# taintpro98/rnd-semantic-segmentation

Measured on AMD Instinct MI355X. Metric: train images/sec at 769x769 bf16 (DeepLabV2-ResNet101 + ASPP), higher is better.
Workload: dtype bf16; 1 GPU; train_src.py DeepLabV2-R101 bf16, 769x769 synthetic Cityscapes crops, batch 8 per GPU, 1xMI355X; global_batch=8, parallelism=dp1, weights=formula (synthetic), hip_graph_replay=False

## Files before the change

### rnd_semantic_segmentation_amd/csrc/pack_aspp.hip

```cpp
#include "mi_common.h"

namespace {

__global__ void pack_fwd_kernel(const float* __restrict__ w, __bf16* __restrict__ wp, int O, int I, int T) {
    const long idx = (long)blockIdx.x * blockDim.x + threadIdx.x;
    if (idx >= (long)O * I) return;
    const long plane = (long)O * I;
    for (int t = 0; t < T; ++t) wp[t * plane + idx] = (__bf16)w[idx * T + t];
}

__global__ void pack_dgrad_kernel(const float* __restrict__ w, const float* __restrict__ scale, __bf16* __restrict__ wp, int O, int I, int T) {
    const long idx = (long)blockIdx.x * blockDim.x + threadIdx.x;
    if (idx >= (long)O * I) return;
    const int i = (int)(idx / O), o = (int)(idx - (long)i * O);
    const float s = scale ? scale[o] : 1.f;
    const long plane = (long)O * I;
    const float* src = w + ((long)o * I + i) * T;
    for (int t = 0; t < T; ++t) wp[t * plane + idx] = (__bf16)(src[t] * s);
}

__global__ void aspp_pack_fwd_kernel(const float* __restrict__ w4, __bf16* __restrict__ wall, int C, int K) {
    const long idx = (long)blockIdx.x * blockDim.x + threadIdx.x;
    const long total = 36L * MI_ASPP_ZGW * C;
    if (idx >= total) return;
// ... 9 lines not shown

__global__ void aspp_pack_dgrad_kernel(const float* __restrict__ w4, __bf16* __restrict__ wallT, int C, int K) {
    const long idx = (long)blockIdx.x * blockDim.x + threadIdx.x;
    const long total = (long)C * MI_ASPP_KPAD;
    if (idx >= total) return;
    const int c = (int)(idx / MI_ASPP_KPAD), k = (int)(idx - (long)c * MI_ASPP_KPAD);
    float v = 0.f;
    if (k < 36 * K) {
        const int g = k / K, n = k - g * K;
        const int r = g / 9, tap = g - r * 9;
        v = w4[(((long)r * K + n) * C + c) * 9 + tap];
    }
    wallT[idx] = (__bf16)v;
}

constexpr int PACK_TILES = 4;
__global__ __launch_bounds__(256) void pack_multi_kernel(const float* __restrict__ wflat, const float* __restrict__ sflat, __bf16* __restrict__ wp,
                                                         __bf16* __restrict__ wpt, const long* __restrict__ table, int n_desc) {
    __shared__ float tile[32][32 * 9 + 1];
    int lo = 0, hi = n_desc - 1;
    while (lo < hi) {
        const int mid = (lo + hi + 1) >> 1;
        if (table[mid * 8 + 7] <= (long)blockIdx.x) lo = mid; else hi = mid - 1;
    }
    const long* d = table + lo * 8;
    const int O = (int)d[4], I = (int)d[5], T = (int)d[6];
    const int tiles_i = (I + 31) >> 5, groups_i = (tiles_i + PACK_TILES - 1) / PACK_TILES;
    const int local = (int)((long)blockIdx.x - d[7]);
    const int ot = local / groups_i;
    const int o0 = ot * 32, it0 = (local - ot * groups_i) * PACK_TILES;
    if (o0 >= O) return;
    const int no = min(32, O - o0);
    const int tid = threadIdx.x, lane = tid & 63, wave = tid >> 6;
    const long plane = (long)O * I;
    const int c = tid & 31, r = tid >> 5;
    const float sc = (d[3] >= 0 && d[1] >= 0 && c < no) ? sflat[d[1] + o0 + c] : 1.f;
    for (int it = it0; it < it0 + PACK_TILES && it < tiles_i; ++it) {
        const int i0 = it * 32;
        const int ni = min(32, I - i0);
        const int rowlen = ni * T;
        if (it != it0) __syncthreads();
        for (int o = wave; o < no; o += 4) {
            const float* src = wflat + d[0] + ((long)(o0 + o) * I + i0) * T;
            for (int e = lane; e < rowlen; e += 64) tile[o][e] = src[e];
        }
        __syncthreads();
        if (c < ni) {
            for (int k = 0; k < 4; ++k) {
                const int o = r + 8 * k;
                if (o >= no) break;
                __bf16* f = wp + d[2] + (long)(o0 + o) * I + i0 + c;
                for (int t = 0; t < T; ++t) f[t * plane] = (__bf16)tile[o][c * T + t];
            }
        }
        if (d[3] >= 0 && c < no) {
            for (int k = 0; k < 4; ++k) {
                const int i = r + 8 * k;
                if (i >= ni) break;
                __bf16* b = wpt + d[3] + (long)(i0 + i) * O + o0 + c;
                for (int t = 0; t < T; ++t) b[t * plane] = (__bf16)(tile[c][i * T + t] * sc);
            }
        }
    }
}

struct Rates { int d[4]; };

__global__ void aspp_col2im_kernel(const float* __restrict__ z, const float* __restrict__ bias4, float* __restrict__ low,
                                   int B, int H, int W, int K, Rates rates) {
    const long idx = (long)blockIdx.x * blockDim.x + threadIdx.x;
    const long M = (long)B * H * W;
    if (idx >= M * MI_ASPP_ZGW) return;
    const long m = idx / MI_ASPP_ZGW;
    const int n = (int)(idx - m * MI_ASPP_ZGW);
    if (n >= K) return;
// ... 149 lines not shown
    MI_CHECK_LAUNCH("mi_pack_weight_fwd");
    return MI_OK;
}

extern "C" int mi_pack_weight_dgrad(const float* w, const float* scale_o, void* wp, int O, int I, int ksize, void* stream) {
    MI_REQUIRE(w && wp && O > 0 && I > 0 && ksize > 0, "mi_pack_weight_dgrad: bad argument");
    hipLaunchKernelGGL(pack_dgrad_kernel, dim3(nblk((long)O * I, 256)), dim3(256), 0, (hipStream_t)stream, w, scale_o, (__bf16*)wp, O, I,
                       ksize * ksize);
    MI_CHECK_LAUNCH("mi_pack_weight_dgrad");
    return MI_OK;
}

extern "C" int mi_pack_weights_multi(const float* wflat, const float* sflat, void* wp, void* wpt, const int64_t* table_dev, int n_desc,
                                     int total_blocks, void* stream) {
    MI_REQUIRE(wflat && wp && table_dev && n_desc > 0 && total_blocks > 0, "mi_pack_weights_multi: bad argument");
    hipLaunchKernelGGL(pack_multi_kernel, dim3(total_blocks), dim3(256), 0, (hipStream_t)stream, wflat, sflat, (__bf16*)wp, (__bf16*)wpt,
                       (const long*)table_dev, n_desc);
    MI_CHECK_LAUNCH("mi_pack_weights_multi");
    return MI_OK;
}

extern "C" int mi_aspp_pack_fwd(const float* w4, void* wall, int C, int K, void* stream) {
    MI_REQUIRE(w4 && wall && C > 0 && K > 0 && K < MI_ASPP_ZGW, "mi_aspp_pack_fwd: bad argument (K=%d must be < 20)", K);
    hipLaunchKernelGGL(aspp_pack_fwd_kernel, dim3(nblk(36L * MI_ASPP_ZGW * C, 256)), dim3(256), 0, (hipStream_t)stream, w4, (__bf16*)wall, C, K);
    MI_CHECK_LAUNCH("mi_aspp_pack_fwd");
    return MI_OK;
}

extern "C" int mi_aspp_pack_dgrad(const float* w4, void* wallT, int C, int K, void* stream) {
    MI_REQUIRE(w4 && wallT && C > 0 && K > 0 && 36 * K <= MI_ASPP_KPAD, "mi_aspp_pack_dgrad: bad argument");
    hipLaunchKernelGGL(aspp_pack_dgrad_kernel, dim3(nblk((long)C * MI_ASPP_KPAD, 256)), dim3(256), 0, (hipStream_t)stream, w4, (__bf16*)wallT, C, K);
// ... 38 lines not shown
```

### rnd_semantic_segmentation_amd/csrc/stem.hip

```cpp
#include "mi_common.h"

namespace {

__global__ void stem_pool_fwd_kernel(const bf16x8* __restrict__ y, const float* __restrict__ scale, const float* __restrict__ shift,
                                     bf16x8* __restrict__ pool, uint8_t* __restrict__ idx, int B, int Hc, int Wc, int C8, int Hp, int Wp) {
    const long id = (long)blockIdx.x * blockDim.x + threadIdx.x;
    if (id >= (long)B * Hp * Wp * C8) return;
    const int c8 = (int)(id % C8);
    const int wo = (int)((id / C8) % Wp), ho = (int)((id / ((long)C8 * Wp)) % Hp), b = (int)(id / ((long)C8 * Wp * Hp));
    float sc[8], sh[8], best[8];
    int bi[8];
#pragma unroll
    for (int e = 0; e < 8; ++e) {
        sc[e] = scale[c8 * 8 + e];
        sh[e] = shift[c8 * 8 + e];
        best[e] = -3.0e38f;
        bi[e] = 9;
    }
#pragma unroll
    for (int ky = 0; ky < 3; ++ky) {
        const int h = 2 * ho - 1 + ky;
        if ((unsigned)h >= (unsigned)Hc) continue;
#pragma unroll
        for (int kx = 0; kx < 3; ++kx) {
// ... 38 lines not shown
            const bf16x8 g = dpool[p];
            const uint2 ib = *reinterpret_cast<const uint2*>(idx + p * 8);
#pragma unroll
            for (int e = 0; e < 8; ++e) {
                const unsigned byte = ((e < 4 ? ib.x : ib.y) >> (8 * (e & 3))) & 0xffu;
                if ((int)byte == tap) acc[e] += (float)g[e];
            }
        }
    }
    bf16x8 o;
#pragma unroll
    for (int e = 0; e < 8; ++e) o[e] = (__bf16)(acc[e] * scale[c8 * 8 + e]);
    dy[id] = o;
}

}

extern "C" int mi_stem_pool_fwd(const void* y, const float* scale, const float* shift, void* pool, uint8_t* idx, int B, int Hc, int Wc, int C,
                                int Hp, int Wp, void* stream) {
    MI_REQUIRE(y && scale && shift && pool && idx && B > 0 && Hc > 0 && Wc > 0 && C > 0 && C % 8 == 0, "mi_stem_pool_fwd: bad argument");
    MI_REQUIRE(Hp == (Hc + 2 - 3) / 2 + 1 && Wp == (Wc + 2 - 3) / 2 + 1, "mi_stem_pool_fwd: pooled size must be that of a 3x3/2/1 max-pool");
    MI_REQUIRE(mi_aligned16(y) && mi_aligned16(pool) && ((uintptr_t)idx & 7) == 0, "mi_stem_pool_fwd: alignment");
    const long n = (long)B * Hp * Wp * (C / 8);
    hipLaunchKernelGGL(stem_pool_fwd_kernel, dim3((unsigned)((n + 255) / 256)), dim3(256), 0, (hipStream_t)stream, (const bf16x8*)y, scale, shift,
                       (bf16x8*)pool, idx, B, Hc, Wc, C / 8, Hp, Wp);
    MI_CHECK_LAUNCH("mi_stem_pool_fwd");
    return MI_OK;
}

extern "C" int mi_stem_pool_bwd(const void* dpool, const uint8_t* idx, const float* scale, void* dy, int B, int Hc, int Wc, int C, int Hp, int Wp,
                                void* stream) {
    MI_REQUIRE(dpool && idx && scale && dy && B > 0 && Hc > 0 && Wc > 0 && C > 0 && C % 8 == 0, "mi_stem_pool_bwd: bad argument");
    MI_REQUIRE(Hp == (Hc + 2 - 3) / 2 + 1 && Wp == (Wc + 2 - 3) / 2 + 1, "mi_stem_pool_bwd: pooled size must be that of a 3x3/2/1 max-pool");
    MI_REQUIRE(mi_aligned16(dpool) && mi_aligned16(dy) && ((uintptr_t)idx & 7) == 0, "mi_stem_pool_bwd: alignment");
    const long n = (long)B * Hc * Wc * (C / 8);
    hipLaunchKernelGGL(stem_pool_bwd_kernel, dim3((unsigned)((n + 255) / 256)), dim3(256), 0, (hipStream_t)stream, (const bf16x8*)dpool, idx, scale,
                       (bf16x8*)dy, B, Hc, Wc, C / 8, Hp, Wp);
    MI_CHECK_LAUNCH("mi_stem_pool_bwd");
    return MI_OK;
}

namespace {
__global__ __launch_bounds__(256) void stem_im2col_kernel(const __bf16* __restrict__ x, bf16x8* __restrict__ col, int B, int H, int W, int Ho, int Wo,
                                                          int groups) {
    const int in_row = blockIdx.x * 256 + threadIdx.x;
    if (in_row >= Wo * groups) return;
    const int wo = in_row / groups, kg = in_row - wo * groups;
    const int ho = blockIdx.y % Ho, b = blockIdx.y / Ho;
    int k = kg * 8;
    int c = k / 49, r = k - c * 49, ky = r / 7, kx = r - ky * 7;
    const __bf16* img = x + (long)b * H * W * 3;
    bf16x8 v;
#pragma unroll
    for (int e = 0; e < 8; ++e) {
        __bf16 val = (__bf16)0.f;
        if (k + e < 147) {
            const int h = 2 * ho - 3 + ky, w = 2 * wo - 3 + kx;
            if ((unsigned)h < (unsigned)H && (unsigned)w < (unsigned)W) val = img[((long)h * W + w) * 3 + c];
        }
        v[e] = val;
        if (++kx == 7) {
            kx = 0;
            if (++ky == 7) {
                ky = 0;
                ++c;
            }
        }
    }
    col[((long)blockIdx.y * Wo + wo) * groups + kg] = v;
}
}

extern "C" int mi_stem_im2col(const void* x_bf16_nhwc, void* col_bf16, int B, int H, int W, int Ho, int Wo, int ncols, void* stream) {
    MI_REQUIRE(x_bf16_nhwc && col_bf16 && B > 0 && H > 0 && W > 0, "mi_stem_im2col: bad argument");
    MI_REQUIRE(ncols >= 152 && ncols % 8 == 0 && ncols <= 256, "mi_stem_im2col: ncols=%d (a multiple of 8 in [152, 256])", ncols);
    MI_REQUIRE(Ho == (H + 6 - 7) / 2 + 1 && Wo == (W + 6 - 7) / 2 + 1, "mi_stem_im2col: output size must be that of a 7x7/2/3 conv");
    MI_REQUIRE(mi_aligned16(col_bf16), "mi_stem_im2col: alignment");
    MI_REQUIRE((long)B * Ho < 65536, "mi_stem_im2col: B * Ho = %ld exceeds the grid", (long)B * Ho);
    hipLaunchKernelGGL(stem_im2col_kernel, dim3((unsigned)((Wo * (ncols / 8) + 255) / 256), (unsigned)(B * Ho)), dim3(256), 0, (hipStream_t)stream,
                       (const __bf16*)x_bf16_nhwc, (bf16x8*)col_bf16, B, H, W, Ho, Wo, ncols / 8);
    MI_CHECK_LAUNCH("mi_stem_im2col");
    return MI_OK;
}
```

### rnd_semantic_segmentation_amd/csrc/upsample_ce.hip

```cpp
#include "mi_common.h"

namespace {

constexpr int KMAX = 32;

struct Axis {
    float scale, off;
    int n_in, n_out;
    __device__ __forceinline__ float srcf(int dst) const {
        const float f = scale * ((float)dst + off) - off;
        return f < 0.f ? 0.f : f;
    }
    __device__ __forceinline__ void src(int dst, int& i0, int& i1, float& lam) const {
        const float f = srcf(dst);
        i0 = (int)f;
        if (i0 > n_in - 1) i0 = n_in - 1;
        i1 = (i0 < n_in - 1) ? i0 + 1 : i0;
        lam = f - (float)i0;
    }
    __device__ __forceinline__ int first_with_i0_ge(int c) const {
        if (c <= 0) return 0;
        if (scale <= 0.f) return n_out;
        if (c > n_in - 1) return n_out;
        int d = (int)((float)c / scale) - 2;
// ... 138 lines not shown
    const float* p = logits + b * K * HW + pix;
    float* d = dlogits + b * K * HW + pix;
    if (lab == ignore_index || lab < 0 || lab >= K) {
        for (int k = 0; k < K; ++k) d[k * HW] = 0.f;
        return;
    }
    const float inv = grad_scale / loss_out[1];
    float mx = p[0];
    for (int k = 1; k < K; ++k) mx = fmaxf(mx, p[k * HW]);
    float se = 0.f;
    for (int k = 0; k < K; ++k) se += __expf(p[k * HW] - mx);
    const float rse = 1.f / se;
    for (int k = 0; k < K; ++k) d[k * HW] = (__expf(p[k * HW] - mx) * rse - (k == lab ? 1.f : 0.f)) * inv;
}

constexpr int JT = 32;

template <int KT>
__global__ __launch_bounds__(256) void upce_pass1_kernel(const float* __restrict__ low, const int64_t* __restrict__ labels,
                                                         float* __restrict__ partial, float* __restrict__ tmp, int B, int Krt, Axis ay,
                                                         Axis ax, int ignore_index, int npx_max, unsigned* __restrict__ bad, int jt_cols) {
    const int K = KT > 0 ? KT : Krt;
    constexpr int KR = KT > 0 ? KT : KMAX;
    extern __shared__ __attribute__((aligned(16))) float sh[];
    float* dbuf = sh;
    float* lam = sh + (long)npx_max * K;
    int* x0s = reinterpret_cast<int*>(lam + npx_max);
    float* red = reinterpret_cast<float*>(x0s + npx_max);
    int* pstart = reinterpret_cast<int*>(red + 512);
    float* vrow = red + 512 + JT + 4;
    const int H = ay.n_out, W = ax.n_out, h = ay.n_in, w = ax.n_in;
    const int jt = blockIdx.x, y = blockIdx.y, b = blockIdx.z;
    const int j0 = jt * jt_cols, j1 = min(w, j0 + jt_cols);
    const int xa = ax.first_with_i0_ge(j0 - 1), xb = ax.first_with_i0_ge(j1);
    const int npx = xb - xa;
    int y0, y1;
    float ly;
    ay.src(y, y0, y1, ly);
    const float* row0 = low + ((long)b * h + y0) * w * K;
    const float* row1 = low + ((long)b * h + y1) * w * K;
    const int cbase = max(j0 - 1, 0), ncol = min(j1, w - 1) - cbase + 1;
    if (threadIdx.x < j1 - j0 + 2) pstart[threadIdx.x] = ax.first_with_i0_ge(j0 - 1 + (int)threadIdx.x) - xa;
    for (int e = threadIdx.x; e < ncol * K; e += 256) {
        const long o = (long)cbase * K + e;
        vrow[e] = (1.f - ly) * row0[o] + ly * row1[o];
    }
    __syncthreads();
    float loss = 0.f, cnt = 0.f;
    for (int px = threadIdx.x; px < npx; px += 256) {
        const int x = xa + px;
        int x0, x1;
        float lx;
        ax.src(x, x0, x1, lx);
        lam[px] = lx;
        const long lab = labels[((long)b * H + y) * W + x];
        float* d = dbuf + (long)px * K;
        if (x0 >= j0) count_bad_label(lab, K, ignore_index, bad);
        if (lab == ignore_index || lab < 0 || lab >= K) {
            for (int k = 0; k < K; ++k) d[k] = 0.f;
            continue;
        }
        const float* c0 = vrow + (x0 - cbase) * K;
        const float* c1 = vrow + (x1 - cbase) * K;
        float v[KR];
        float mx = -3.0e38f;
#pragma unroll
        for (int k = 0; k < KR; ++k) {
            if (k < K) {
                v[k] = (1.f - lx) * c0[k] + lx * c1[k];
                mx = fmaxf(mx, v[k]);
// ... 8 lines not shown
                se += v[k];
            }
        }
        const float rse = 1.f / se;
#pragma unroll
        for (int k = 0; k < KR; ++k) {
            if (k < K) d[k] = v[k] * rse - (k == lab ? 1.f : 0.f);
        }
        if (x0 >= j0) {
            loss += __logf(se) - picked;
            cnt += 1.f;
        }
    }
    __syncthreads();
    if (tmp) {
        const int nj = j1 - j0;
        for (int item = threadIdx.x; item < nj * K; item += 256) {
            const int jj = item / K, k = item - jj * K;
            const int j = j0 + jj;
            float s = 0.f;
            const int p0 = max(pstart[jj], 0), p1 = min(max(pstart[jj + 1], 0), npx), p2 = min(pstart[jj + 2], npx);
            for (int px = p0; px < p1; ++px) s += (0.f + lam[px]) * dbuf[(long)px * K + k];
            const bool edge = j == w - 1;
            for (int px = p1; px < p2; ++px) s += ((1.f - lam[px]) + (edge ? lam[px] : 0.f)) * dbuf[(long)px * K + k];
            tmp[(((long)b * H + y) * w + j) * K + k] = s;
        }
    }
    block_sum2(loss, cnt, red);
    if (threadIdx.x == 0) {
        const long pidx = ((long)b * H + y) * gridDim.x + jt;
        partial[2 * pidx] = loss;
        partial[2 * pidx + 1] = cnt;
    }
}

__global__ void upce_pass2_kernel(const float* __restrict__ tmp, const float* __restrict__ loss_out, float* __restrict__ dlow, int B, int K,
                                  Axis ay, int w, float grad_scale) {
    const long idx = (long)blockIdx.x * blockDim.x + threadIdx.x;
    const int H = ay.n_out, h = ay.n_in;
    const long per_row = (long)w * K;
    if (idx >= (long)B * h * per_row) return;
    const long jk = idx % per_row;
    const int i = (int)((idx / per_row) % h), b = (int)(idx / (per_row * h));
// ... 312 lines not shown
}

extern "C" int mi_upsample_ce_ex(const float* low, const int64_t* labels, float* loss_out, float* dlow, int B, int h, int w, int K, int H, int W,
                                 int ignore_index, float grad_scale, int align_corners, void* workspace, size_t workspace_bytes, void* stream) {
    MI_REQUIRE(low && labels && loss_out && workspace, "mi_upsample_ce: null operand");
    MI_REQUIRE(B > 0 && h > 0 && w > 0 && H > 0 && W > 0 && K > 0 && K <= KMAX, "mi_upsample_ce: bad dimension (K <= 32)");
    MI_REQUIRE(H >= h && W >= w, "mi_upsample_ce: only upsampling (H >= h, W >= w) is supported");
    MI_REQUIRE(H <= 65535 && B <= 65535, "mi_upsample_ce: grid dimension overflow");
    if (workspace_bytes < mi_upsample_ce_workspace(B, h, w, K, H, W)) return mi_set_error(MI_ENOMEM, "mi_upsample_ce: workspace too small");
    const Axis ay = make_axis(h, H, align_corners), ax = make_axis(w, W, align_corners);
    const int jt_cols = pick_jt(w, W);
    const int tiles = (w + jt_cols - 1) / jt_cols;
    float* partial = (float*)workspace;
    const size_t poff = (((size_t)B * H * tiles * 2 * sizeof(float)) + 255) & ~(size_t)255;
    float* tmp = dlow ? (float*)((char*)workspace + poff) : nullptr;
    const int npx_max = pass1_npx_max(ax, jt_cols);
    const size_t lds = (size_t)npx_max * K * 4 + (size_t)npx_max * 8 + 512 * 4 + (JT + 4) * 4 + (size_t)(JT + 2) * K * 4;
    MI_REQUIRE(lds <= 160 * 1024, "mi_upsample_ce: upsample factor too large for one LDS tile (%zu B)", lds);
    static std::atomic<uint64_t> lds_set[2];
    mi_allow_dynamic_lds((const void*)upce_pass1_kernel<19>, MI_LDS_MAX, lds_set[0]);
    mi_allow_dynamic_lds((const void*)upce_pass1_kernel<0>, MI_LDS_MAX, lds_set[1]);
    unsigned* bad = reinterpret_cast<unsigned*>(loss_out + 3);
    if (hipMemsetAsync(bad, 0, sizeof(unsigned), (hipStream_t)stream) != hipSuccess) return mi_set_error(MI_EHIP, "mi_upsample_ce: memset");
    if (K == 19)
        hipLaunchKernelGGL(upce_pass1_kernel<19>, dim3(tiles, H, B), dim3(256), lds, (hipStream_t)stream, low, labels, partial, tmp, B, K, ay,
                           ax, ignore_index, npx_max, bad, jt_cols);
    else
        hipLaunchKernelGGL(upce_pass1_kernel<0>, dim3(tiles, H, B), dim3(256), lds, (hipStream_t)stream, low, labels, partial, tmp, B, K, ay,
                           ax, ignore_index, npx_max, bad, jt_cols);
    MI_CHECK_LAUNCH("mi_upsample_ce pass1");
    hipLaunchKernelGGL(ce_finalize_kernel, dim3(1), dim3(256), 0, (hipStream_t)stream, (const float*)partial, B * H * tiles, loss_out);
    MI_CHECK_LAUNCH("mi_upsample_ce finalize");
    if (dlow) {
        hipLaunchKernelGGL(upce_pass2_kernel, dim3(nblk((long)B * h * w * K, 256)), dim3(256), 0, (hipStream_t)stream, (const float*)tmp, loss_out,
                           dlow, B, K, ay, w, grad_scale);
        MI_CHECK_LAUNCH("mi_upsample_ce pass2");
    }
    return MI_OK;
}

extern "C" int mi_upsample_softmax(const float* low, float* probs, uint8_t* pred, int B, int h, int w, int K, int H, int W, void* stream) {
    MI_REQUIRE(low && probs && B > 0 && h > 0 && w > 0 && H > 0 && W > 0 && K > 0 && K <= KMAX, "mi_upsample_softmax: bad argument (K <= 32)");
    hipLaunchKernelGGL(upsample_softmax_kernel, dim3(nblk((long)B * H * W, 256)), dim3(256), 0, (hipStream_t)stream, low, probs, pred, B, K,
                       make_axis(h, H), make_axis(w, W));
// ... 69 lines not shown
```

### rnd_semantic_segmentation_amd/host/engine.py

```python
import contextlib
import os

import torch

from .. import kernels as K
from . import arch


class FlatStore:

    ALIGN = 64

    def __init__(self, named_params, device):
        self.names = [n for n, _ in named_params]
        self.params = [p for _, p in named_params]
        self.offsets = []
        off = 0
        for p in self.params:
            self.offsets.append(off)
            off += -(-p.numel() // self.ALIGN) * self.ALIGN
        self.total = off
        self.data = torch.zeros(off, dtype=torch.float32, device=device)
        self.grad = torch.zeros(off, dtype=torch.float32, device=device)
        self.written = set()
# ... 317 lines not shown
                out = self._fwd_conv(a2, rts[2], True, res=idn)
            x = out
        return x, saved, xbits

    @staticmethod
    def _wgrad(dy, xin, rt, batch=None):
        c = rt.spec
        dw, acc = grad_slot(rt.weight)
        K.conv_wgrad(dy, xin, dw, c.k, c.stride, c.pad, c.dil, scale=rt.scale, accumulate=acc, batch=batch)

    @staticmethod
    def _dgrad(dy, rt, in_hw, res=None, bits=None):
        c = rt.spec
        return K.conv_gemm(dy, rt.wpt, in_hw, c.k, c.stride, c.pad, c.dil, K.GATHER_DGRAD, res=res, bits=bits)

    def backward(self, saved, fbits, dfeat, need_dx):
        g = K.relu_mask(dfeat, fbits)
        store = getattr(self.convs[0].weight, "_mi_store", None)
        sched = WgradScheduler.on(dfeat.device)
        chain = self.chain_mode() in ("all", "bwd") and self._chain_fits(dfeat)
        ga2_ahead = None
        for bi in range(len(self.blocks) - 1, -1, -1):
            blk, rts = self.blocks[bi]
            x, a1, a2, xb, b1, b2 = saved[bi]
            first = bi == 0
            hw_in = (x.shape[1], x.shape[2])
            hw_mid = (a1.shape[1], a1.shape[2])
            wb = K.WgradBatch() if K.PROFILE is None else None
            sched.run(lambda: self._wgrad(g, a2, rts[2], wb), g, a2)
            if ga2_ahead is not None:
                ga2, ga2_ahead = ga2_ahead, None
            else:
# ... 263 lines not shown
    @staticmethod
    def forward(ctx, x, weight, scale, shift):
        y, saved = stem_conv_forward(x, weight)
        pool, idx = K.stem_pool_fwd(y, scale, shift)
        ctx.save_for_backward(idx, scale, *saved)
        ctx.conv_hw = (y.shape[1], y.shape[2])
        return pool

    @staticmethod
    def backward(ctx, dpool):
        idx, scale = ctx.saved_tensors[:2]
        dy = K.stem_pool_bwd(dpool.contiguous(), idx, scale, ctx.conv_hw)
        return None, stem_conv_wgrad(dy, ctx.saved_tensors[2:]), None, None


class StagesFn(torch.autograd.Function):

    @staticmethod
    def forward(ctx, x, eng, *weights):
        train = any(ctx.needs_input_grad)
        eng.prepare(train)
        feat, saved, fbits = eng.forward(x, save=train)
        ctx.eng, ctx.saved, ctx.fbits = eng, saved, fbits
        return feat

    @staticmethod
    def backward(ctx, dfeat):
        dfeat = dfeat.contiguous()
        dx = ctx.eng.backward(ctx.saved, ctx.fbits, dfeat, ctx.needs_input_grad[0])
        ctx.saved = ctx.fbits = None
        return (dx, None) + (None,) * (len(ctx.needs_input_grad) - 2)


class AsppEngine:

    def __init__(self, owner, rates, num_classes, in_channels):
        self.owner, self.rates, self.K, self.C = owner, tuple(int(r) for r in rates), num_classes, in_channels
        self.wall = self.wallT = None
        self._sig = None
        self._have_dgrad = False

    @staticmethod
    def _room(t):
        return t.untyped_storage().nbytes() // t.element_size() - t.storage_offset()
# ... 18 lines not shown
        store = getattr(ws[0], "_mi_store", None)
        sig = (store.generation if store is not None else -1, sum(w._version for w in ws), ws[0].data_ptr())
        if sig != self._sig or (train and not self._have_dgrad):
            self.wall = K.aspp_pack_fwd(w4, out=self.wall)
            if train:
                self.wallT = K.aspp_pack_dgrad(w4, out=self.wallT)
            self._sig = sig
            self._have_dgrad = train

    def forward(self, x):
        B, h, w, _ = x.shape
        z = K.conv_gemm(x, self.wall, (h, w), zsplit=K.ASPP_ZGW, flop_cols=self.K)
        b4, _ = self._b4()
        return K.aspp_col2im(z, b4, B, h, w, self.K, self.rates)

    def backward(self, x, dlow, need_dx, msk=None):
        h, w = x.shape[1], x.shape[2]
        g = K.aspp_im2col(dlow, self.rates)
        w4, ws = self._w4()
        b4, bs = self._b4()
        sched = WgradScheduler.on(x.device)

        def weight_and_bias_grads():
            slots = [grad_slot(p) for p in ws]
            n = ws[0].numel()
            base = slots[0][0].data_ptr()
            stacked = all(s[0].data_ptr() == base + 4 * n * i for i, s in enumerate(slots)) and len({s[1] for s in slots}) == 1
            if stacked:
                dw4 = torch.as_strided(slots[0][0], (4,) + tuple(ws[0].shape), (n,) + tuple(ws[0].stride()))
                K.conv_wgrad(g, x, dw4, out_map=1, ncls=self.K, accumulate=slots[0][1])
            else:
                dw4 = torch.empty((4,) + tuple(ws[0].shape), dtype=torch.float32, device=x.device)
                K.conv_wgrad(g, x, dw4, out_map=1, ncls=self.K)
                for i, (slot, acc) in enumerate(slots):
                    slot.add_(dw4[i]) if acc else slot.copy_(dw4[i])
            bslots = [grad_slot(p) for p in bs]
            bbase = bslots[0][0].data_ptr()
            if all(s[0].data_ptr() == bbase + 4 * self.K * i for i, s in enumerate(bslots)) and len({s[1] for s in bslots}) == 1:
                K.aspp_bias_grad(dlow, torch.as_strided(bslots[0][0], (4, self.K), (self.K, 1)), accumulate=bslots[0][1])
            else:
                db4 = torch.empty((4, self.K), dtype=torch.float32, device=x.device)
                K.aspp_bias_grad(dlow, db4)
                for i, (slot, acc) in enumerate(bslots):
                    slot.add_(db4[i]) if acc else slot.copy_(db4[i])

        sched.run(weight_and_bias_grads, g, x, dlow)
        dx = K.conv_gemm(g, self.wallT, (h, w), msk=msk, flop_cols=36 * self.K) if need_dx else None
        sched.join()
        store = getattr(ws[0], "_mi_store", None)
        if store is not None and store.grad_hooks:
            for hook in store.grad_hooks:
                hook(store, 0, store.total)
        return dx


class AsppFn(torch.autograd.Function):

    @staticmethod
    def forward(ctx, x, eng, *params):
        train = any(ctx.needs_input_grad)
        eng.prepare(train)
        ctx.eng, ctx.x = eng, (x if train else None)
        return eng.forward(x)

    @staticmethod
    def backward(ctx, dlow):
        dx = ctx.eng.backward(ctx.x, dlow.contiguous().float(), ctx.needs_input_grad[0])
        ctx.x = None
        return (dx, None) + (None,) * (len(ctx.needs_input_grad) - 2)


class AsppLossFn(torch.autograd.Function):

    @staticmethod
    def forward(ctx, x, labels, eng, ignore_index, temperature, *params):
        train = any(ctx.needs_input_grad)
        eng.prepare(train)
        low = eng.forward(x)
        eng.last_low = low
        if temperature != 1.0:
            loss_out, dlow = K.upsample_ce(low * (1.0 / temperature), labels, want_grad=train, grad_scale=1.0 / temperature,
                                           ignore_index=ignore_index)
        else:
            loss_out, dlow = K.upsample_ce(low, labels, want_grad=train, ignore_index=ignore_index)
        ctx.eng, ctx.x, ctx.dlow = eng, (x if train else None), dlow
        ctx.loss_out = eng.last_loss_out = loss_out
        bad = getattr(eng, "bad_labels", None)
        if bad is None or bad.device != loss_out.device:
            bad = eng.bad_labels = torch.zeros(1, dtype=torch.float32, device=loss_out.device)
        bad.add_(loss_out[2:3])
        return loss_out[0].clone()

    @staticmethod
    def backward(ctx, gout):
        dlow = ctx.dlow * gout
        dx = ctx.eng.backward(ctx.x, dlow, ctx.needs_input_grad[0])
        ctx.x = ctx.dlow = None
        return (dx, None, None, None, None) + (None,) * (len(ctx.needs_input_grad) - 5)


class UpsampleFn(torch.autograd.Function):

    @staticmethod
    def forward(ctx, low, size):
        ctx.hw = (low.shape[1], low.shape[2])
        return K.upsample_ac_fwd(low, tuple(int(s) for s in size))

    @staticmethod
    def backward(ctx, dup):
        return K.upsample_ac_bwd(dup.contiguous(), ctx.hw), None

# ... 18 lines not shown
```

### rnd_semantic_segmentation_amd/kernels.py

```python
import collections
import ctypes

import torch

from . import _lib
from ._lib import check

EPI_SCALE_BIAS, EPI_RESIDUAL, EPI_RELU, EPI_MASK, EPI_OUT_F32, EPI_ZSPLIT, EPI_WRITE_MASK, EPI_BITMASK, EPI_LEAKY = 1, 2, 4, 8, 16, 32, 64, 128, 256
GATHER_FWD, GATHER_DGRAD = 0, 1
ASPP_ZGW, ASPP_KPAD = 20, 704


def _stream():
    return ctypes.c_void_p(torch.cuda.current_stream().cuda_stream)


PROFILE = None


def _timed(name, flops, launch, tag=None):
    if PROFILE is None:
        return launch()
    e0, e1 = torch.cuda.Event(enable_timing=True), torch.cuda.Event(enable_timing=True)
    e0.record()
# ... 591 lines not shown


def sgd_step(p, g, buf, lr, momentum, weight_decay):
    for t, n in ((p, "p"), (g, "g"), (buf, "buf")):
        _chk(t, torch.float32, n)
    check(_lib.lib().mi_sgd_step(_p(p), _p(g), _p(buf), p.numel(), float(lr), float(momentum), float(weight_decay), _stream()),
          "mi_sgd_step")


def sgd_step_dev(p, g, buf, hyper):
    for t, n in ((p, "p"), (g, "g"), (buf, "buf"), (hyper, "hyper")):
        _chk(t, torch.float32, n)
    check(_lib.lib().mi_sgd_step_dev(_p(p), _p(g), _p(buf), p.numel(), _p(hyper), _stream()), "mi_sgd_step_dev")


def relu_mask(x, msk, out=None):
    _chk(x, torch.bfloat16, "x")
    bits = msk.dtype == torch.int16
    _chk(msk, torch.int16 if bits else torch.bfloat16, "msk")
    if out is None:
        out = torch.empty_like(x)
    check(_lib.lib().mi_relu_mask(_p(x), _p(msk), _p(out), x.numel(), int(bits), _stream()), "mi_relu_mask")
    return out


def frozen_bn_fold(w, b, mean, var):
    for t in (w, b, mean, var):
        _chk(t, torch.float32, "bn buffer")
    scale, shift = torch.empty_like(w), torch.empty_like(w)
    check(_lib.lib().mi_frozen_bn_fold(_p(w), _p(b), _p(mean), _p(var), _p(scale), _p(shift), w.numel(), _stream()),
          "mi_frozen_bn_fold")
# ... 181 lines not shown
```

Measured before the change: 298.5 images/s.

## Fuse boundary ReLU mask into ASPP dgrad and retile pack, pool-bwd, im2col, CE kernels

Several independent changes land together. The backbone-to-ASPP boundary ReLU mask is passed into the ASPP dgrad GEMM epilogue, so the separate relu_mask pass over dfeat is skipped. The weight-pack kernel uses wider dynamic-LDS tiles with 16-byte vectorized loads and stores. Stem max-pool backward gets an LDS-tiled kernel, stem im2col stages input rows in LDS, and the upsample-CE pass1 processes two items per thread and balances column tiles. The boundary mask relies on a pointer/version registry that adds Python bookkeeping and may silently fall back if tensors are not matched.

Result: no change. 298.2 images/s (-0.1%).

```diff
diff --git a/rnd_semantic_segmentation_amd/csrc/pack_aspp.hip b/rnd_semantic_segmentation_amd/csrc/pack_aspp.hip
--- a/rnd_semantic_segmentation_amd/csrc/pack_aspp.hip
+++ b/rnd_semantic_segmentation_amd/csrc/pack_aspp.hip
@@ -47,10 +47,14 @@
     wallT[idx] = (__bf16)v;
 }
 
-constexpr int PACK_TILES = 4;
+constexpr int PACK_BI = 128;
+constexpr int PACK_ROW = 64 * 9 + 1;
+constexpr int PACK_LDS = 32 * PACK_ROW * (int)sizeof(float);
+__device__ __forceinline__ bool dev_aligned16(const void* p) { return (reinterpret_cast<uintptr_t>(p) & 15) == 0; }
 __global__ __launch_bounds__(256) void pack_multi_kernel(const float* __restrict__ wflat, const float* __restrict__ sflat, __bf16* __restrict__ wp,
                                                          __bf16* __restrict__ wpt, const long* __restrict__ table, int n_desc) {
-    __shared__ float tile[32][32 * 9 + 1];
+    extern __shared__ __attribute__((aligned(16))) float pack_lds[];
+    float (*tile)[PACK_ROW] = reinterpret_cast<float (*)[PACK_ROW]>(pack_lds);
     int lo = 0, hi = n_desc - 1;
     while (lo < hi) {
         const int mid = (lo + hi + 1) >> 1;
@@ -58,40 +62,88 @@
     }
     const long* d = table + lo * 8;
     const int O = (int)d[4], I = (int)d[5], T = (int)d[6];
-    const int tiles_i = (I + 31) >> 5, groups_i = (tiles_i + PACK_TILES - 1) / PACK_TILES;
+    const int groups_i = (I + PACK_BI - 1) / PACK_BI;
     const int local = (int)((long)blockIdx.x - d[7]);
     const int ot = local / groups_i;
-    const int o0 = ot * 32, it0 = (local - ot * groups_i) * PACK_TILES;
-    if (o0 >= O) return;
-    const int no = min(32, O - o0);
+    const int o0 = ot * 32, ib0 = (local - ot * groups_i) * PACK_BI;
+    if (o0 >= O || T < 1 || T > 72) return;
+    const int no = min(32, O - o0), iend = min(I, ib0 + PACK_BI);
+    const int CI = T <= 4 ? PACK_BI : max(8, ((PACK_ROW - 1) / T) & ~7);
     const int tid = threadIdx.x, lane = tid & 63, wave = tid >> 6;
     const long plane = (long)O * I;
-    const int c = tid & 31, r = tid >> 5;
-    const float sc = (d[3] >= 0 && d[1] >= 0 && c < no) ? sflat[d[1] + o0 + c] : 1.f;
-    for (int it = it0; it < it0 + PACK_TILES && it < tiles_i; ++it) {
-        const int i0 = it * 32;
-        const int ni = min(32, I - i0);
+    const bool has_t = d[3] >= 0;
+    __bf16* wpb = wp + d[2];
+    __bf16* wptb = has_t ? wpt + d[3] : nullptr;
+    const float* sp = (has_t && d[1] >= 0) ? sflat + d[1] + o0 : nullptr;
+    const bool vec_f = I % 8 == 0 && dev_aligned16(wpb);
+    const bool vec_b = has_t && O % 8 == 0 && dev_aligned16(wptb);
+    for (int i0 = ib0; i0 < iend; i0 += CI) {
+        const int ni = min(CI, iend - i0);
         const int rowlen = ni * T;
-        if (it != it0) __syncthreads();
+        if (i0 != ib0) __syncthreads();
         for (int o = wave; o < no; o += 4) {
             const float* src = wflat + d[0] + ((long)(o0 + o) * I + i0) * T;
-            for (int e = lane; e < rowlen; e += 64) tile[o][e] = src[e];
+            float* dst = tile[o];
+            if (dev_aligned16(src)) {
+                const int n4 = rowlen >> 2;
+                for (int q = lane; q < n4; q += 64) {
+                    const f32x4 v = *reinterpret_cast<const f32x4*>(src + 4 * q);
+                    dst[4 * q] = v[0];
+                    dst[4 * q + 1] = v[1];
+                    dst[4 * q + 2] = v[2];
+                    dst[4 * q + 3] = v[3];
+                }
+                for (int e = 4 * n4 + lane; e < rowlen; e += 64) dst[e] = src[e];
+            } else {
+                for (int e = lane; e < rowlen; e += 64) dst[e] = src[e];
+            }
         }
         __syncthreads();
-        if (c < ni) {
-            for (int k = 0; k < 4; ++k) {
-                const int o = r + 8 * k;
-                if (o >= no) break;
-                __bf16* f = wp + d[2] + (long)(o0 + o) * I + i0 + c;
+        if (vec_f) {
+            const int cpr = CI >> 3, nc = ni >> 3;
+            for (int p = tid; p < 32 * cpr; p += 256) {
+                const int o = p / cpr, ic = p - o * cpr;
+                if (o >= no || ic >= nc) continue;
+                const float* s = tile[o] + ic * 8 * T;
+                __bf16* f = wpb + (long)(o0 + o) * I + i0 + 8 * ic;
+                for (int t = 0; t < T; ++t) {
+                    bf16x8 v;
+#pragma unroll
+                    for (int e = 0; e < 8; ++e) v[e] = (__bf16)s[e * T + t];
+                    *reinterpret_cast<bf16x8*>(f + t * plane) = v;
+                }
+            }
+        } else {
+            for (int p = tid; p < 32 * CI; p += 256) {
+                const int o = p / CI, c = p - o * CI;
+                if (o >= no || c >= ni) continue;
+                __bf16* f = wpb + (long)(o0 + o) * I + i0 + c;
                 for (int t = 0; t < T; ++t) f[t * plane] = (__bf16)tile[o][c * T + t];
             }
         }
-        if (d[3] >= 0 && c < no) {
-            for (int k = 0; k < 4; ++k) {
-                const int i = r + 8 * k;
-                if (i >= ni) break;
-                __bf16* b = wpt + d[3] + (long)(i0 + i) * O + o0 + c;
-                for (int t = 0; t < T; ++t) b[t * plane] = (__bf16)(tile[c][i * T + t] * sc);
+        if (vec_b) {
+            const int nc = no >> 3;
+            for (int p = tid; p < 4 * CI; p += 256) {
+                const int i = p >> 2, oc = p & 3;
+                if (i >= ni || oc >= nc) continue;
+                float sc[8];
+#pragma unroll
+                for (int e = 0; e < 8; ++e) sc[e] = sp ? sp[8 * oc + e] : 1.f;
+                __bf16* g = wptb + (long)(i0 + i) * O + o0 + 8 * oc;
+                for (int t = 0; t < T; ++t) {
+                    bf16x8 v;
+#pragma unroll
+                    for (int e = 0; e < 8; ++e) v[e] = (__bf16)(tile[8 * oc + e][i * T + t] * sc[e]);
+                    *reinterpret_cast<bf16x8*>(g + t * plane) = v;
+                }
+            }
+        } else if (has_t) {
+            for (int p = tid; p < 32 * CI; p += 256) {
+                const int i = p >> 5, c = p & 31;
+                if (i >= ni || c >= no) continue;
+                const float sc = sp ? sp[c] : 1.f;
+                __bf16* g = wptb + (long)(i0 + i) * O + o0 + c;
+                for (int t = 0; t < T; ++t) g[t * plane] = (__bf16)(tile[c][i * T + t] * sc);
             }
         }
     }
@@ -271,7 +323,9 @@
 extern "C" int mi_pack_weights_multi(const float* wflat, const float* sflat, void* wp, void* wpt, const int64_t* table_dev, int n_desc,
                                      int total_blocks, void* stream) {
     MI_REQUIRE(wflat && wp && table_dev && n_desc > 0 && total_blocks > 0, "mi_pack_weights_multi: bad argument");
-    hipLaunchKernelGGL(pack_multi_kernel, dim3(total_blocks), dim3(256), 0, (hipStream_t)stream, wflat, sflat, (__bf16*)wp, (__bf16*)wpt,
+    static std::atomic<uint64_t> lds_set;
+    mi_allow_dynamic_lds((const void*)pack_multi_kernel, PACK_LDS, lds_set);
+    hipLaunchKernelGGL(pack_multi_kernel, dim3(total_blocks), dim3(256), PACK_LDS, (hipStream_t)stream, wflat, sflat, (__bf16*)wp, (__bf16*)wpt,
                        (const long*)table_dev, n_desc);
     MI_CHECK_LAUNCH("mi_pack_weights_multi");
     return MI_OK;
diff --git a/rnd_semantic_segmentation_amd/csrc/stem.hip b/rnd_semantic_segmentation_amd/csrc/stem.hip
--- a/rnd_semantic_segmentation_amd/csrc/stem.hip
+++ b/rnd_semantic_segmentation_amd/csrc/stem.hip
@@ -76,6 +76,61 @@
     dy[id] = o;
 }
 
+constexpr int POOL_TH = 4, POOL_TW = 64, POOL_PH = POOL_TH / 2 + 1, POOL_PW = POOL_TW / 2 + 1, POOL_C8 = 8;
+__global__ __launch_bounds__(256) void stem_pool_bwd_tile_kernel(const bf16x8* __restrict__ dpool, const uint8_t* __restrict__ idx,
+                                                                 const float* __restrict__ scale, bf16x8* __restrict__ dy, int Hc, int Wc, int C8,
+                                                                 int Hp, int Wp) {
+    __shared__ bf16x8 sg[POOL_PH * POOL_PW * POOL_C8];
+    __shared__ uint2 si[POOL_PH * POOL_PW * POOL_C8];
+    const int w0 = blockIdx.x * POOL_TW, h0 = blockIdx.y * POOL_TH, b = blockIdx.z;
+    const int ho0 = h0 >> 1, wo0 = w0 >> 1;
+    const int rowv = POOL_PW * C8;
+    for (int v = threadIdx.x; v < POOL_PH * rowv; v += 256) {
+        const int pr = v / rowv, rem = v - pr * rowv;
+        const int pc = rem / C8, c8 = rem - pc * C8;
+        const int ho = ho0 + pr, wo = wo0 + pc;
+        bf16x8 g;
+#pragma unroll
+        for (int e = 0; e < 8; ++e) g[e] = (__bf16)0.f;
+        uint2 ib = make_uint2(0xffffffffu, 0xffffffffu);
+        if (ho < Hp && wo < Wp) {
+            const long p = (((long)b * Hp + ho) * Wp + wo) * C8 + c8;
+            g = dpool[p];
+            ib = *reinterpret_cast<const uint2*>(idx + p * 8);
+        }
+        sg[v] = g;
+        si[v] = ib;
+    }
+    __syncthreads();
+    const int tilev = POOL_TW * C8;
+    for (int v = threadIdx.x; v < POOL_TH * tilev; v += 256) {
+        const int hh = v / tilev, rem = v - hh * tilev;
+        const int ww = rem / C8, c8 = rem - ww * C8;
+        const int h = h0 + hh, w = w0 + ww;
+        if (h >= Hc || w >= Wc) continue;
+        float acc[8] = {0.f, 0.f, 0.f, 0.f, 0.f, 0.f, 0.f, 0.f};
+        const int ho_lo = h >> 1, ho_hi = (h + 1) >> 1, wo_lo = w >> 1, wo_hi = (w + 1) >> 1;
+        for (int ho = ho_lo; ho <= ho_hi; ++ho) {
+            const int ky = h - (2 * ho - 1);
+            for (int wo = wo_lo; wo <= wo_hi; ++wo) {
+                const int tap = ky * 3 + (w - (2 * wo - 1));
+                const int s = ((ho - ho0) * POOL_PW + (wo - wo0)) * C8 + c8;
+                const bf16x8 g = sg[s];
+                const uint2 ib = si[s];
+#pragma unroll
+                for (int e = 0; e < 8; ++e) {
+                    const unsigned byte = ((e < 4 ? ib.x : ib.y) >> (8 * (e & 3))) & 0xffu;
+                    if ((int)byte == tap) acc[e] += (float)g[e];
+                }
+            }
+        }
+        bf16x8 o;
+#pragma unroll
+        for (int e = 0; e < 8; ++e) o[e] = (__bf16)(acc[e] * scale[c8 * 8 + e]);
+        dy[(((long)b * Hc + h) * Wc + w) * C8 + c8] = o;
+    }
+}
+
 }
 
 extern "C" int mi_stem_pool_fwd(const void* y, const float* scale, const float* shift, void* pool, uint8_t* idx, int B, int Hc, int Wc, int C,
@@ -96,40 +151,80 @@
     MI_REQUIRE(Hp == (Hc + 2 - 3) / 2 + 1 && Wp == (Wc + 2 - 3) / 2 + 1, "mi_stem_pool_bwd: pooled size must be that of a 3x3/2/1 max-pool");
     MI_REQUIRE(mi_aligned16(dpool) && mi_aligned16(dy) && ((uintptr_t)idx & 7) == 0, "mi_stem_pool_bwd: alignment");
     const long n = (long)B * Hc * Wc * (C / 8);
-    hipLaunchKernelGGL(stem_pool_bwd_kernel, dim3((unsigned)((n + 255) / 256)), dim3(256), 0, (hipStream_t)stream, (const bf16x8*)dpool, idx, scale,
-                       (bf16x8*)dy, B, Hc, Wc, C / 8, Hp, Wp);
+    const unsigned strips = (unsigned)((Hc + POOL_TH - 1) / POOL_TH);
+    if (C / 8 <= POOL_C8 && strips <= 65535u && B <= 65535)
+        hipLaunchKernelGGL(stem_pool_bwd_tile_kernel, dim3((unsigned)((Wc + POOL_TW - 1) / POOL_TW), strips, (unsigned)B), dim3(256), 0,
+                           (hipStream_t)stream, (const bf16x8*)dpool, idx, scale, (bf16x8*)dy, Hc, Wc, C / 8, Hp, Wp);
+    else
+        hipLaunchKernelGGL(stem_pool_bwd_kernel, dim3((unsigned)((n + 255) / 256)), dim3(256), 0, (hipStream_t)stream, (const bf16x8*)dpool, idx,
+                           scale, (bf16x8*)dy, B, Hc, Wc, C / 8, Hp, Wp);
     MI_CHECK_LAUNCH("mi_stem_pool_bwd");
     return MI_OK;
 }
 
 namespace {
+constexpr int IM2COL_SEG = 128;
+constexpr int IM2COL_ROW = ((2 * IM2COL_SEG + 5) * 3 + 7 + 7) / 8 * 8;
 __global__ __launch_bounds__(256) void stem_im2col_kernel(const __bf16* __restrict__ x, bf16x8* __restrict__ col, int B, int H, int W, int Ho, int Wo,
-                                                          int groups) {
-    const int in_row = blockIdx.x * 256 + threadIdx.x;
-    if (in_row >= Wo * groups) return;
-    const int wo = in_row / groups, kg = in_row - wo * groups;
+                                                          int groups, int seg) {
+    __shared__ __attribute__((aligned(16))) __bf16 rows[7 * IM2COL_ROW];
     const int ho = blockIdx.y % Ho, b = blockIdx.y / Ho;
-    int k = kg * 8;
-    int c = k / 49, r = k - c * 49, ky = r / 7, kx = r - ky * 7;
-    const __bf16* img = x + (long)b * H * W * 3;
-    bf16x8 v;
-#pragma unroll
-    for (int e = 0; e < 8; ++e) {
-        __bf16 val = (__bf16)0.f;
-        if (k + e < 147) {
-            const int h = 2 * ho - 3 + ky, w = 2 * wo - 3 + kx;
-            if ((unsigned)h < (unsigned)H && (unsigned)w < (unsigned)W) val = img[((long)h * W + w) * 3 + c];
-        }
-        v[e] = val;
-        if (++kx == 7) {
-            kx = 0;
-            if (++ky == 7) {
-                ky = 0;
-                ++c;
-            }
-        }
-    }
-    col[((long)blockIdx.y * Wo + wo) * groups + kg] = v;
+    const int wo_first = blockIdx.x * seg, nwo = min(seg, Wo - wo_first);
+    const int w_first = 2 * wo_first - 3, span = (2 * nwo + 5) * 3;
+    const long mis = (long)((reinterpret_cast<uintptr_t>(x) >> 1) & 7);
+    constexpr int CH = IM2COL_ROW / 8;
+    for (int item = threadIdx.x; item < 7 * CH; item += 256) {
+        const int r = item / CH, i = item - r * CH;
+        const int h = 2 * ho - 3 + r;
+        const long first = (((long)b * H + h) * W + w_first) * 3;
+        const int shift = (int)((first + mis) & 7);
+        if (8 * i >= shift + span) continue;
+        const long e0 = first - shift + 8 * i;
+        long lo = 0, hi = 0;
+        if ((unsigned)h < (unsigned)H) {
+            lo = (((long)b * H + h) * W + max(w_first, 0)) * 3;
+            hi = (((long)b * H + h) * W + min(w_first + 2 * nwo + 5, W)) * 3;
+        }
+        bf16x8 v;
+        if (e0 >= lo && e0 + 8 <= hi) {
+            v = *reinterpret_cast<const bf16x8*>(x + e0);
+        } else {
+#pragma unroll
+            for (int e = 0; e < 8; ++e) v[e] = (e0 + e >= lo && e0 + e < hi) ? x[e0 + e] : (__bf16)0.f;
+        }
+        *reinterpret_cast<bf16x8*>(rows + r * IM2COL_ROW + 8 * i) = v;
+    }
+    __syncthreads();
+    const int per_pass = 256 / groups;
+    const int kg = threadIdx.x % groups, wl = threadIdx.x / groups;
+    if (wl >= per_pass) return;
+    int off[8];
+    {
+        int k = kg * 8;
+        int c = k / 49, r = k - c * 49, ky = r / 7, kx = r - ky * 7;
+#pragma unroll
+        for (int e = 0; e < 8; ++e) {
+            off[e] = -1;
+            if (k + e < 147) {
+                const long first = (((long)b * H + (2 * ho - 3 + ky)) * W + w_first) * 3;
+                off[e] = ky * IM2COL_ROW + (int)((first + mis) & 7) + kx * 3 + c;
+            }
+            if (++kx == 7) {
+                kx = 0;
+                if (++ky == 7) {
+                    ky = 0;
+                    ++c;
+                }
+            }
+        }
+    }
+    bf16x8* dst = col + ((long)blockIdx.y * Wo + wo_first) * groups + kg;
+    for (int j = wl; j < nwo; j += per_pass) {
+        bf16x8 v;
+#pragma unroll
+        for (int e = 0; e < 8; ++e) v[e] = off[e] >= 0 ? rows[off[e] + 6 * j] : (__bf16)0.f;
+        dst[(long)j * groups] = v;
+    }
 }
 }
 
@@ -139,8 +234,9 @@
     MI_REQUIRE(Ho == (H + 6 - 7) / 2 + 1 && Wo == (W + 6 - 7) / 2 + 1, "mi_stem_im2col: output size must be that of a 7x7/2/3 conv");
     MI_REQUIRE(mi_aligned16(col_bf16), "mi_stem_im2col: alignment");
     MI_REQUIRE((long)B * Ho < 65536, "mi_stem_im2col: B * Ho = %ld exceeds the grid", (long)B * Ho);
-    hipLaunchKernelGGL(stem_im2col_kernel, dim3((unsigned)((Wo * (ncols / 8) + 255) / 256), (unsigned)(B * Ho)), dim3(256), 0, (hipStream_t)stream,
-                       (const __bf16*)x_bf16_nhwc, (bf16x8*)col_bf16, B, H, W, Ho, Wo, ncols / 8);
+    const int nseg = (Wo + IM2COL_SEG - 1) / IM2COL_SEG, seg = (Wo + nseg - 1) / nseg;
+    hipLaunchKernelGGL(stem_im2col_kernel, dim3((unsigned)((Wo + seg - 1) / seg), (unsigned)(B * Ho)), dim3(256), 0, (hipStream_t)stream,
+                       (const __bf16*)x_bf16_nhwc, (bf16x8*)col_bf16, B, H, W, Ho, Wo, ncols / 8, seg);
     MI_CHECK_LAUNCH("mi_stem_im2col");
     return MI_OK;
 }
diff --git a/rnd_semantic_segmentation_amd/csrc/upsample_ce.hip b/rnd_semantic_segmentation_amd/csrc/upsample_ce.hip
--- a/rnd_semantic_segmentation_amd/csrc/upsample_ce.hip
+++ b/rnd_semantic_segmentation_amd/csrc/upsample_ce.hip
@@ -176,26 +176,47 @@
     for (int k = 0; k < K; ++k) d[k * HW] = (__expf(p[k * HW] - mx) * rse - (k == lab ? 1.f : 0.f)) * inv;
 }
 
+__device__ __forceinline__ void block_sum2_thread0(float& a, float& b, float* red) {
+    const int t = threadIdx.x;
+    red[t] = a;
+    red[256 + t] = b;
+    __syncthreads();
+    if (t < 64) {
+        float va = (red[t] + red[t + 128]) + (red[t + 64] + red[t + 192]);
+        float vb = (red[256 + t] + red[256 + t + 128]) + (red[256 + t + 64] + red[256 + t + 192]);
+#pragma unroll
+        for (int w = 32; w > 0; w >>= 1) {
+            va += __shfl_down(va, w, 64);
+            vb += __shfl_down(vb, w, 64);
+        }
+        a = va;
+        b = vb;
+    }
+}
+
 constexpr int JT = 32;
 
 template <int KT>
 __global__ __launch_bounds__(256) void upce_pass1_kernel(const float* __restrict__ low, const int64_t* __restrict__ labels,
                                                          float* __restrict__ partial, float* __restrict__ tmp, int B, int Krt, Axis ay,
-                                                         Axis ax, int ignore_index, int npx_max, unsigned* __restrict__ bad, int jt_cols) {
+                                                         Axis ax, int ignore_index, int npx_max, unsigned* __restrict__ bad, int jt_base, int jt_rem) {
     const int K = KT > 0 ? KT : Krt;
     constexpr int KR = KT > 0 ? KT : KMAX;
     extern __shared__ __attribute__((aligned(16))) float sh[];
     float* dbuf = sh;
     float* lam = sh + (long)npx_max * K;
-    int* x0s = reinterpret_cast<int*>(lam + npx_max);
-    float* red = reinterpret_cast<float*>(x0s + npx_max);
+    float* oml = lam + npx_max;
+    float* red = oml + npx_max;
     int* pstart = reinterpret_cast<int*>(red + 512);
     float* vrow = red + 512 + JT + 4;
     const int H = ay.n_out, W = ax.n_out, h = ay.n_in, w = ax.n_in;
     const int jt = blockIdx.x, y = blockIdx.y, b = blockIdx.z;
-    const int j0 = jt * jt_cols, j1 = min(w, j0 + jt_cols);
+    const int j0 = jt * jt_base + min(jt, jt_rem), j1 = j0 + jt_base + (jt < jt_rem ? 1 : 0);
     const int xa = ax.first_with_i0_ge(j0 - 1), xb = ax.first_with_i0_ge(j1);
     const int npx = xb - xa;
+    const int64_t* lrow = labels + ((long)b * H + y) * W + xa;
+    long lab_first = 0;
+    if ((int)threadIdx.x < npx) lab_first = lrow[threadIdx.x];
     int y0, y1;
     float ly;
     ay.src(y, y0, y1, ly);
@@ -214,8 +235,9 @@
         int x0, x1;
         float lx;
         ax.src(x, x0, x1, lx);
-        lam[px] = lx;
-        const long lab = labels[((long)b * H + y) * W + x];
+        lam[px] = 0.f + lx;
+        oml[px] = (1.f - lx) + (x0 == w - 1 ? lx : 0.f);
+        const long lab = px < 256 ? lab_first : (long)lrow[px];
         float* d = dbuf + (long)px * K;
         if (x0 >= j0) count_bad_label(lab, K, ignore_index, bad);
         if (lab == ignore_index || lab < 0 || lab >= K) {
@@ -254,19 +276,44 @@
     }
     __syncthreads();
     if (tmp) {
-        const int nj = j1 - j0;
-        for (int item = threadIdx.x; item < nj * K; item += 256) {
-            const int jj = item / K, k = item - jj * K;
-            const int j = j0 + jj;
-            float s = 0.f;
-            const int p0 = max(pstart[jj], 0), p1 = min(max(pstart[jj + 1], 0), npx), p2 = min(pstart[jj + 2], npx);
-            for (int px = p0; px < p1; ++px) s += (0.f + lam[px]) * dbuf[(long)px * K + k];
-            const bool edge = j == w - 1;
-            for (int px = p1; px < p2; ++px) s += ((1.f - lam[px]) + (edge ? lam[px] : 0.f)) * dbuf[(long)px * K + k];
-            tmp[(((long)b * H + y) * w + j) * K + k] = s;
-        }
-    }
-    block_sum2(loss, cnt, red);
+        const int nitems = (j1 - j0) * K;
+        float* trow = tmp + (((long)b * H + y) * w + j0) * K;
+        for (int item = threadIdx.x; item < nitems; item += 512) {
+            const int item2 = item + 256;
+            const bool two = item2 < nitems;
+            const int jja = item / K, ka = item - jja * K;
+            const int jjb = two ? item2 / K : jja, kb = two ? item2 - jjb * K : ka;
+            const int a0 = max(pstart[jja], 0), a1 = min(max(pstart[jja + 1], 0), npx), a2 = min(pstart[jja + 2], npx);
+            const int b0 = max(pstart[jjb], 0), b1 = min(max(pstart[jjb + 1], 0), npx), b2 = min(pstart[jjb + 2], npx);
+            float sa = 0.f, sb = 0.f;
+            int pa = a0, pb = b0;
+            while (pa < a1 || pb < b1) {
+                if (pa < a1) {
+                    sa += lam[pa] * dbuf[(long)pa * K + ka];
+                    ++pa;
+                }
+                if (pb < b1) {
+                    sb += lam[pb] * dbuf[(long)pb * K + kb];
+                    ++pb;
+                }
+            }
+            pa = a1;
+            pb = b1;
+            while (pa < a2 || pb < b2) {
+                if (pa < a2) {
+                    sa += oml[pa] * dbuf[(long)pa * K + ka];
+                    ++pa;
+                }
+                if (pb < b2) {
+                    sb += oml[pb] * dbuf[(long)pb * K + kb];
+                    ++pb;
+                }
+            }
+            trow[item] = sa;
+            if (two) trow[item2] = sb;
+        }
+    }
+    block_sum2_thread0(loss, cnt, red);
     if (threadIdx.x == 0) {
         const long pidx = ((long)b * H + y) * gridDim.x + jt;
         partial[2 * pidx] = loss;
@@ -609,7 +656,8 @@
     float* partial = (float*)workspace;
     const size_t poff = (((size_t)B * H * tiles * 2 * sizeof(float)) + 255) & ~(size_t)255;
     float* tmp = dlow ? (float*)((char*)workspace + poff) : nullptr;
-    const int npx_max = pass1_npx_max(ax, jt_cols);
+    const int jt_base = w / tiles, jt_rem = w % tiles;
+    const int npx_max = pass1_npx_max(ax, jt_base + (jt_rem ? 1 : 0));
     const size_t lds = (size_t)npx_max * K * 4 + (size_t)npx_max * 8 + 512 * 4 + (JT + 4) * 4 + (size_t)(JT + 2) * K * 4;
     MI_REQUIRE(lds <= 160 * 1024, "mi_upsample_ce: upsample factor too large for one LDS tile (%zu B)", lds);
     static std::atomic<uint64_t> lds_set[2];
@@ -619,10 +667,10 @@
     if (hipMemsetAsync(bad, 0, sizeof(unsigned), (hipStream_t)stream) != hipSuccess) return mi_set_error(MI_EHIP, "mi_upsample_ce: memset");
     if (K == 19)
         hipLaunchKernelGGL(upce_pass1_kernel<19>, dim3(tiles, H, B), dim3(256), lds, (hipStream_t)stream, low, labels, partial, tmp, B, K, ay,
-                           ax, ignore_index, npx_max, bad, jt_cols);
+                           ax, ignore_index, npx_max, bad, jt_base, jt_rem);
     else
         hipLaunchKernelGGL(upce_pass1_kernel<0>, dim3(tiles, H, B), dim3(256), lds, (hipStream_t)stream, low, labels, partial, tmp, B, K, ay,
-                           ax, ignore_index, npx_max, bad, jt_cols);
+                           ax, ignore_index, npx_max, bad, jt_base, jt_rem);
     MI_CHECK_LAUNCH("mi_upsample_ce pass1");
     hipLaunchKernelGGL(ce_finalize_kernel, dim3(1), dim3(256), 0, (hipStream_t)stream, (const float*)partial, B * H * tiles, loss_out);
     MI_CHECK_LAUNCH("mi_upsample_ce finalize");
diff --git a/rnd_semantic_segmentation_amd/host/engine.py b/rnd_semantic_segmentation_amd/host/engine.py
--- a/rnd_semantic_segmentation_amd/host/engine.py
+++ b/rnd_semantic_segmentation_amd/host/engine.py
@@ -355,8 +355,8 @@
         c = rt.spec
         return K.conv_gemm(dy, rt.wpt, in_hw, c.k, c.stride, c.pad, c.dil, K.GATHER_DGRAD, res=res, bits=bits)
 
-    def backward(self, saved, fbits, dfeat, need_dx):
-        g = K.relu_mask(dfeat, fbits)
+    def backward(self, saved, fbits, dfeat, need_dx, masked=False):
+        g = dfeat if masked else K.relu_mask(dfeat, fbits)
         store = getattr(self.convs[0].weight, "_mi_store", None)
         sched = WgradScheduler.on(dfeat.device)
         chain = self.chain_mode() in ("all", "bwd") and self._chain_fits(dfeat)
@@ -650,6 +650,50 @@
         return None, stem_conv_wgrad(dy, ctx.saved_tensors[2:]), None, None
 
 
+_BOUNDARY = {}
+_MASKED = {}
+_BOUNDARY_CAP = 8
+
+
+def _same_memory(a, b):
+    return (a.data_ptr() == b.data_ptr() and a.shape == b.shape and a.dtype == b.dtype and a.device == b.device
+            and a.is_contiguous() and b.is_contiguous())
+
+
+def _capped_put(table, key, value):
+    table.pop(key, None)
+    while len(table) >= _BOUNDARY_CAP:
+        table.pop(next(iter(table)))
+    table[key] = value
+
+
+def boundary_register(feat, bits):
+    _capped_put(_BOUNDARY, feat.data_ptr(), (feat, bits))
+
+
+def boundary_release(bits):
+    for k in [k for k, v in _BOUNDARY.items() if v[1] is bits]:
+        del _BOUNDARY[k]
+
+
+def boundary_bits(x):
+    e = _BOUNDARY.get(x.data_ptr())
+    if e is None or not _same_memory(x, e[0]) or x._version != e[0]._version:
+        return None
+    return e[1]
+
+
+def mark_masked(dx, bits):
+    _capped_put(_MASKED, dx.data_ptr(), (dx, dx._version, bits))
+
+
+def take_masked(dfeat, bits):
+    e = _MASKED.get(dfeat.data_ptr())
+    for k in [k for k, v in _MASKED.items() if v[2] is bits]:
+        del _MASKED[k]
+    return e is not None and e[2] is bits and _same_memory(dfeat, e[0]) and dfeat._version == e[1]
+
+
 class StagesFn(torch.autograd.Function):
 
     @staticmethod
@@ -658,12 +702,15 @@
         eng.prepare(train)
         feat, saved, fbits = eng.forward(x, save=train)
         ctx.eng, ctx.saved, ctx.fbits = eng, saved, fbits
+        if train and fbits is not None:
+            boundary_register(feat, fbits)
         return feat
 
     @staticmethod
     def backward(ctx, dfeat):
         dfeat = dfeat.contiguous()
-        dx = ctx.eng.backward(ctx.saved, ctx.fbits, dfeat, ctx.needs_input_grad[0])
+        boundary_release(ctx.fbits)
+        dx = ctx.eng.backward(ctx.saved, ctx.fbits, dfeat, ctx.needs_input_grad[0], masked=take_masked(dfeat, ctx.fbits))
         ctx.saved = ctx.fbits = None
         return (dx, None) + (None,) * (len(ctx.needs_input_grad) - 2)
 
@@ -712,7 +759,7 @@
         b4, _ = self._b4()
         return K.aspp_col2im(z, b4, B, h, w, self.K, self.rates)
 
-    def backward(self, x, dlow, need_dx, msk=None):
+    def backward(self, x, dlow, need_dx, msk=None, bits=None):
         h, w = x.shape[1], x.shape[2]
         g = K.aspp_im2col(dlow, self.rates)
         w4, ws = self._w4()
@@ -743,7 +790,9 @@
                     slot.add_(db4[i]) if acc else slot.copy_(db4[i])
 
         sched.run(weight_and_bias_grads, g, x, dlow)
-        dx = K.conv_gemm(g, self.wallT, (h, w), msk=msk, flop_cols=36 * self.K) if need_dx else None
+        dx = K.conv_gemm(g, self.wallT, (h, w), msk=msk, bits=bits, flop_cols=36 * self.K) if need_dx else None
+        if dx is not None and bits is not None:
+            mark_masked(dx, bits)
         sched.join()
         store = getattr(ws[0], "_mi_store", None)
         if store is not None and store.grad_hooks:
@@ -763,7 +812,7 @@
 
     @staticmethod
     def backward(ctx, dlow):
-        dx = ctx.eng.backward(ctx.x, dlow.contiguous().float(), ctx.needs_input_grad[0])
+        dx = ctx.eng.backward(ctx.x, dlow.contiguous().float(), ctx.needs_input_grad[0], bits=boundary_bits(ctx.x) if ctx.needs_input_grad[0] else None)
         ctx.x = None
         return (dx, None) + (None,) * (len(ctx.needs_input_grad) - 2)
 
@@ -792,7 +841,7 @@
     @staticmethod
     def backward(ctx, gout):
         dlow = ctx.dlow * gout
-        dx = ctx.eng.backward(ctx.x, dlow, ctx.needs_input_grad[0])
+        dx = ctx.eng.backward(ctx.x, dlow, ctx.needs_input_grad[0], bits=boundary_bits(ctx.x) if ctx.needs_input_grad[0] else None)
         ctx.x = ctx.dlow = None
         return (dx, None, None, None, None) + (None,) * (len(ctx.needs_input_grad) - 5)
 
diff --git a/rnd_semantic_segmentation_amd/kernels.py b/rnd_semantic_segmentation_amd/kernels.py
--- a/rnd_semantic_segmentation_amd/kernels.py
+++ b/rnd_semantic_segmentation_amd/kernels.py
@@ -629,7 +629,12 @@
     check(_lib.lib().mi_sgd_step_dev(_p(p), _p(g), _p(buf), p.numel(), _p(hyper), _stream()), "mi_sgd_step_dev")
 
 
+RELU_MASK_CALLS = 0
+
+
 def relu_mask(x, msk, out=None):
+    global RELU_MASK_CALLS
+    RELU_MASK_CALLS += 1
     _chk(x, torch.bfloat16, "x")
     bits = msk.dtype == torch.int16
     _chk(msk, torch.int16 if bits else torch.bfloat16, "msk")
```
